# fab-jul/L3C-PyTorch

Measured on AMD Instinct MI355X. Metric: MPix/s encode (net+CDF+AC) on 768x512 RGB, higher is better.
Workload: dtype f32; 1 GPU; L3C 0306_0001 (cr.cf, synthetic seeded checkpoint), batch of 768x512 synthetic RGB per GPU: net forward + fused logistic-mixture CDF head + HIP range coder -> bytes in HBM; checkpoint=calibrated, batch_per_gpu=128, image=768x512, coder_cus=0

## Files before the change

### include/l3c_hip.h

```cpp
#ifndef L3C_HIP_H_
#define L3C_HIP_H_

#include <stdint.h>

#ifdef __cplusplus
extern "C" {
#endif

#define L3C_OK 0
#define L3C_ERR_INVALID_ARG (-1)
#define L3C_ERR_HIP (-2)
#define L3C_ERR_UNSUPPORTED (-3)

#define L3C_ABI_VERSION 4

typedef void *l3c_stream_t;


int l3c_abi_version(void);
#define L3C_BITSTREAM_GENERATION 3
int l3c_bitstream_generation(void);
const char *l3c_last_error(void);
int l3c_device_info(char *name_host, int name_cap, int *num_cu_host, char *arch_host, int arch_cap);

// ... 192 lines not shown
#define L3C_EPI_PIXEL_SHUFFLE 4

typedef struct {
    const float *in;
    int in_cstride, in_coff;
    const float *packed_w;
    const float *bias;
    const float *residual;
    int res_cstride, res_coff;
    float *out;
    int out_cstride, out_coff;
    int B, Hin, Win, Cin, Cout;
    int KS;
    int stride;
    int dilation;
    int epilogue;
} l3c_conv_desc;

int l3c_conv_mfma(const l3c_conv_desc *desc_host, l3c_stream_t stream);
int64_t l3c_conv_wino4_packed_words(int Cout, int Cin);
int l3c_conv_wino4_pack_weights(const float *w_oihw, int Cout, int Cin, float *packed, l3c_stream_t stream);
int l3c_conv_wino4(const l3c_conv_desc *desc_host, l3c_stream_t stream);
int l3c_conv_wino4_phase(const l3c_conv_desc *desc_host, int phase_y, int phase_x, l3c_stream_t stream);
int l3c_conv_wino4_stride2(const l3c_conv_desc *desc_host, l3c_stream_t stream);
int l3c_conv_wino4_set_tiles_per_block(int n);
int64_t l3c_conv_pw_packed_words(int Cout, int Cin);
int l3c_conv_pw_pack_weights(const float *w_oi, int Cout, int Cin, float *packed, l3c_stream_t stream);
int l3c_conv_pw(const l3c_conv_desc *desc_host, l3c_stream_t stream);
int l3c_conv_direct(const l3c_conv_desc *desc_host, l3c_stream_t stream);

int l3c_rgb_head(const float *img, const float *w1, const float *b1, const float *w2, const float *b2,
                 const float *w3, const float *b3, int B, int H, int W, int Cf, float *out, float *shifted_out,
                 l3c_stream_t stream);

int l3c_to_q_quantize(const float *feat, const float *w, const float *b, const float *levels, int64_t B, int64_t HW,
                      int Cf, int C, int L, int16_t *sym, float *bn_q, float *bn, l3c_stream_t stream);

int l3c_dec_head(const float *bn_q, const float *w, const float *b, const float *fuse, int64_t B, int64_t HW, int C,
                 int Cf, float *out, l3c_stream_t stream);

int l3c_meanshift_planar(const float *img, const float *w, const float *b, int64_t B, int64_t HW, float *out,
                         l3c_stream_t stream);
int l3c_rgb_to_u8(const float *x, const float *mean3_host, int64_t B, int64_t HW, uint8_t *out, l3c_stream_t stream);
int l3c_resample_u8(const uint8_t *in, int64_t planes, int H, int W, int axis, int out_size, const int32_t *bounds,
                    const int32_t *kk, int ksize, uint8_t *out, l3c_stream_t stream);
int l3c_u8_to_sym_bn(const uint8_t *in, const float *mean3_host, int64_t B, int64_t HW, int16_t *sym, float *bn,
                     l3c_stream_t stream);

typedef struct {
    const uint8_t *out;
    const uint32_t *nbytes;
    int64_t stride;
    int C, H, W;
} l3c_container_scale;
int l3c_container_write(const l3c_container_scale *scales, int n_scales, int64_t B, const uint16_t *padding,
                        const int64_t *file_offset, uint8_t *dst, l3c_stream_t stream);

int l3c_container_read(const uint8_t *files, const int64_t *src_offset, const int64_t *dst_offset, const uint32_t *nbytes,
                       int64_t n_streams, uint32_t max_nbytes, uint8_t *dst, l3c_stream_t stream);

int l3c_ac_band_intervals(const uint32_t *intervals, int64_t n_streams, int64_t n_sym, int64_t band_len, uint32_t *full_out,
                          uint32_t *last_out, l3c_stream_t stream);

typedef struct {
    const uint8_t *out_full;
    const uint32_t *nbytes_full;
// ... 190 lines not shown
```

### l3c-pytorch_amd/_lib.py

```python
import ctypes
import os

import torch

_HERE = os.path.dirname(os.path.abspath(__file__))
LIB_PATH = os.environ.get('L3C_LIB') or os.path.join(_HERE, 'csrc', 'libl3c_hip.so')

c_i64, c_int, c_vp, c_f32 = ctypes.c_int64, ctypes.c_int, ctypes.c_void_p, ctypes.c_float


class L3CError(RuntimeError):
    pass


class ConvDesc(ctypes.Structure):
    _fields_ = [('inp', c_vp), ('in_cstride', c_int), ('in_coff', c_int),
                ('packed_w', c_vp), ('bias', c_vp),
                ('residual', c_vp), ('res_cstride', c_int), ('res_coff', c_int),
                ('out', c_vp), ('out_cstride', c_int), ('out_coff', c_int),
                ('B', c_int), ('Hin', c_int), ('Win', c_int), ('Cin', c_int), ('Cout', c_int),
                ('KS', c_int), ('stride', c_int), ('dilation', c_int), ('epilogue', c_int)]


class AcGroup(ctypes.Structure):
# ... 141 lines not shown
    'l3c_dmll_cdf_table_parts': (c_int, [c_vp, c_vp, c_vp, c_i64, c_i64, c_int, c_int, c_int, c_int, ctypes.POINTER(TablePart), c_int, c_vp]),
    'l3c_decode_rgb_workspace_bytes': (c_i64, [c_i64, c_i64, c_int, c_int]),
    'l3c_decode_rgb_stats_offset': (c_i64, [c_i64, c_i64, c_int, c_int]),
    'l3c_decode_rgb': (c_int, [ctypes.POINTER(RgbDecodeDesc), c_vp, c_vp]),
    'l3c_decode_rgb_ragged_workspace_bytes': (c_i64, [c_i64, c_i64, c_int, c_int]),
    'l3c_decode_rgb_ragged': (c_int, [ctypes.POINTER(RgbRaggedDesc), c_vp, c_vp]),
    'l3c_dmll_cdf_table_ragged': (c_int, [c_vp, c_vp, c_vp, ctypes.POINTER(RaggedBatch), c_int, c_int, c_int, c_int, ctypes.POINTER(TablePart),
                                          ctypes.POINTER(RaggedPart), c_int, c_vp]),
    'l3c_ac_decode_state_bytes': (c_i64, []),
    'l3c_ac_decode_chunks': (c_int, [ctypes.POINTER(AcDecodePart), c_int, c_vp]),
    'l3c_ac_decode': (c_int, [c_vp, c_i64, c_int, c_vp, c_vp, c_vp, c_i64, c_i64, c_int, c_vp, c_vp]),
    'l3c_cdf_check_monotone': (c_int, [c_vp, c_i64, c_int, c_vp, c_vp]),
    'l3c_dmll_channel_params': (c_int, [c_vp, c_vp, c_i64, c_i64, c_int, c_int, c_int, c_int, c_vp, c_vp, c_vp, c_vp]),
    'l3c_cdf_table_mixture': (c_int, [c_vp, c_vp, c_vp, c_vp, c_i64, c_i64, c_int, c_int, c_vp, c_vp, c_vp]),
    'l3c_dmll_encode_intervals': (c_int, [c_vp, c_vp, c_vp, c_i64, c_i64, c_int, c_int, c_int, c_int, c_vp, c_vp]),
    'l3c_dmll_cdf_table': (c_int, [c_vp, c_vp, c_vp, c_i64, c_i64, c_int, c_int, c_int, c_int, c_i64, c_i64, c_int, c_vp, c_vp, c_vp, c_vp]),
    'l3c_dmll_sample': (c_int, [c_vp, c_vp, c_vp, c_i64, c_i64, c_int, c_int, c_int, c_vp, c_vp]),
    'l3c_dmll_mean': (c_int, [c_vp, c_i64, c_i64, c_int, c_int, c_int, c_f32, c_f32, c_int, c_vp, c_vp]),
    'l3c_dmll_nll': (c_int, [c_vp, c_vp, c_i64, c_i64, c_int, c_int, c_int, c_f32, c_f32, c_int, c_vp, c_vp]),
    'l3c_conv_packed_words': (c_i64, [c_int, c_int, c_int]),
    'l3c_conv_pack_weights': (c_int, [c_vp, c_int, c_int, c_int, c_vp, c_vp]),
    'l3c_conv_mfma': (c_int, [ctypes.POINTER(ConvDesc), c_vp]),
    'l3c_conv_wino4_packed_words': (c_i64, [c_int, c_int]),
    'l3c_conv_wino4_pack_weights': (c_int, [c_vp, c_int, c_int, c_vp, c_vp]),
    'l3c_conv_wino4': (c_int, [ctypes.POINTER(ConvDesc), c_vp]),
    'l3c_conv_wino4_phase': (c_int, [ctypes.POINTER(ConvDesc), c_int, c_int, c_vp]),
    'l3c_conv_wino4_stride2': (c_int, [ctypes.POINTER(ConvDesc), c_vp]),
    'l3c_conv_wino4_set_tiles_per_block': (c_int, [c_int]),
    'l3c_conv_pw_packed_words': (c_i64, [c_int, c_int]),
    'l3c_conv_pw_pack_weights': (c_int, [c_vp, c_int, c_int, c_vp, c_vp]),
    'l3c_conv_pw': (c_int, [ctypes.POINTER(ConvDesc), c_vp]),
    'l3c_conv_direct': (c_int, [ctypes.POINTER(ConvDesc), c_vp]),
    'l3c_rgb_head': (c_int, [c_vp, c_vp, c_vp, c_vp, c_vp, c_vp, c_vp, c_int, c_int, c_int, c_int, c_vp, c_vp, c_vp]),
    'l3c_to_q_quantize': (c_int, [c_vp, c_vp, c_vp, c_vp, c_i64, c_i64, c_int, c_int, c_int, c_vp, c_vp, c_vp, c_vp]),
    'l3c_dec_head': (c_int, [c_vp, c_vp, c_vp, c_vp, c_i64, c_i64, c_int, c_int, c_vp, c_vp]),
    'l3c_meanshift_planar': (c_int, [c_vp, c_vp, c_vp, c_i64, c_i64, c_vp, c_vp]),
    'l3c_rgb_to_u8': (c_int, [c_vp, ctypes.POINTER(c_f32), c_i64, c_i64, c_vp, c_vp]),
    'l3c_resample_u8': (c_int, [c_vp, c_i64, c_int, c_int, c_int, c_int, c_vp, c_vp, c_int, c_vp, c_vp]),
    'l3c_u8_to_sym_bn': (c_int, [c_vp, ctypes.POINTER(c_f32), c_i64, c_i64, c_vp, c_vp, c_vp]),
    'l3c_sym_to_bn': (c_int, [c_vp, c_i64, c_f32, c_f32, c_vp, c_vp]),
    'l3c_net_param_count': (c_int, [ctypes.POINTER(NetConfig)]),
    'l3c_net_param': (c_int, [ctypes.POINTER(NetConfig), c_int, ctypes.c_char_p, c_int, ctypes.POINTER(c_int), ctypes.POINTER(c_i64)]),
    'l3c_net_packed_bytes': (c_i64, [ctypes.POINTER(NetConfig)]),
    'l3c_net_pack_workspace_bytes': (c_i64, [ctypes.POINTER(NetConfig)]),
    'l3c_net_pack': (c_int, [ctypes.POINTER(NetConfig), ctypes.POINTER(c_vp), c_vp, c_i64, c_vp, c_i64, c_vp]),
    'l3c_net_forward_workspace_bytes': (c_i64, [ctypes.POINTER(NetConfig), c_i64, c_int, c_int]),
    'l3c_net_forward': (c_int, [ctypes.POINTER(NetForwardDesc), c_vp]),
    'l3c_net_get_p_workspace_bytes': (c_i64, [ctypes.POINTER(NetConfig), c_i64, c_int, c_int]),
    'l3c_net_get_p': (c_int, [ctypes.POINTER(NetGetPDesc), c_vp]),
    'l3c_container_layout': (c_int, [ctypes.POINTER(ContainerScale), c_int, c_i64, c_i64, c_vp, c_vp, c_vp]),
    'l3c_sym_to_u8': (c_int, [c_vp, c_i64, c_vp, c_vp]),
    'l3c_encode_file_stride': (c_i64, [ctypes.POINTER(NetConfig), c_int, c_int]),
    'l3c_encode_batch_workspace_bytes': (c_i64, [ctypes.POINTER(NetConfig), c_i64, c_int, c_int]),
    'l3c_encode_batch': (c_int, [ctypes.POINTER(EncodeBatchDesc), c_vp]),
    'l3c_decode_plan_bytes': (c_i64, [ctypes.POINTER(NetConfig), c_i64]),
    'l3c_decode_plan': (c_int, [ctypes.POINTER(NetConfig), c_vp, ctypes.POINTER(c_i64), c_i64, c_vp, c_i64, ctypes.POINTER(c_int),
                                ctypes.POINTER(c_int), c_vp]),
    'l3c_decode_batch_workspace_bytes': (c_i64, [ctypes.POINTER(NetConfig), c_vp]),
    'l3c_decode_batch': (c_int, [ctypes.POINTER(DecodeBatchDesc), c_vp, c_vp]),
    'l3c_ac_decode_bands': (c_int, [c_vp, c_int, c_vp, c_vp, c_vp, c_i64, c_i64, c_i64, c_int, c_vp, c_vp]),
    'l3c_container_layout_banded': (c_int, [ctypes.POINTER(BandedScale), c_int, c_i64, c_i64, c_vp, c_vp, c_vp]),
    'l3c_encode_banded_file_stride': (c_i64, [ctypes.POINTER(NetConfig), c_int, c_int, c_int]),
    'l3c_encode_batch_banded_workspace_bytes': (c_i64, [ctypes.POINTER(NetConfig), c_i64, c_int, c_int, c_int]),
    'l3c_encode_batch_banded': (c_int, [ctypes.POINTER(EncodeBatchDesc), c_int, c_vp]),
    'l3c_decode_plan_banded_bytes': (c_i64, [ctypes.POINTER(NetConfig), c_vp, ctypes.POINTER(c_i64), c_i64]),
    'l3c_decode_plan_banded': (c_int, [ctypes.POINTER(NetConfig), c_vp, ctypes.POINTER(c_i64), c_i64, c_vp, c_i64, ctypes.POINTER(c_int),
# ... 135 lines not shown
```

### l3c-pytorch_amd/csrc/conv_small.hip

```cpp
#include "l3c_common.h"

namespace {

typedef float f32x4 __attribute__((ext_vector_type(4)));

constexpr int RH_TH = 8, RH_TW = 32, RH_NT = 4;

__global__ __launch_bounds__(256) void rgb_head_kernel(const float *__restrict__ img, const float *__restrict__ w1,
                                                       const float *__restrict__ b1, const float *__restrict__ w2,
                                                       const float *__restrict__ b2, const float *__restrict__ w3,
                                                       const float *__restrict__ b3, int H, int W, int Cf,
                                                       float *__restrict__ out, float *__restrict__ shifted_out) {
    extern __shared__ __attribute__((aligned(16))) float smem[];
    float *s_w = smem;
    float *s_in = smem + 27 * Cf;
    constexpr int IH = RH_TH + 2, IW = RH_TW + 2;
    const int tid = threadIdx.x;
    const int b = blockIdx.z;
    const int ox0 = blockIdx.x * RH_TW;
    for (int i = tid; i < 27 * Cf; i += 256) {
        const int co = i % Cf, r = i / Cf;
        const int ci = r % 3, tap = r / 3;
        s_w[i] = w3[((size_t)co * 3 + ci) * 9 + tap];
    }
    __syncthreads();
    const int quads = Cf / 4;
    const int q = tid % quads;
    const int pix_per_pass = 256 / quads;
    f32x4 wreg[27];
#pragma unroll
    for (int t = 0; t < 27; ++t) wreg[t] = *reinterpret_cast<const f32x4 *>(&s_w[t * Cf + q * 4]);
    const f32x4 bias = *reinterpret_cast<const f32x4 *>(&b3[q * 4]);
    const size_t plane = (size_t)H * W;
    const float *im = img + (size_t)b * 3 * plane;
    const int Hb = H, Wb = W;
    if (ox0 >= Wb) return;
    for (int nt = 0; nt < RH_NT; ++nt) {
        const int oy0 = (blockIdx.y * RH_NT + nt) * RH_TH;
        if (oy0 >= Hb) break;
        if (nt) __syncthreads();
        for (int i = tid; i < IH * IW; i += 256) {
            const int r = i / IW, c = i % IW;
            const int y = oy0 + r - 1, x = ox0 + c - 1;
            float z[3] = {0.f, 0.f, 0.f};
            if (y >= 0 && y < Hb && x >= 0 && x < Wb) {
                float v[3], u[3];
#pragma unroll
                for (int k = 0; k < 3; ++k) v[k] = im[k * plane + (size_t)y * W + x];
#pragma unroll
                for (int o = 0; o < 3; ++o) u[o] = ((v[0] * w1[o * 3 + 0] + v[1] * w1[o * 3 + 1]) + v[2] * w1[o * 3 + 2]) + b1[o];
#pragma unroll
                for (int o = 0; o < 3; ++o) z[o] = ((u[0] * w2[o * 3 + 0] + u[1] * w2[o * 3 + 1]) + u[2] * w2[o * 3 + 2]) + b2[o];
                if (shifted_out && r >= 1 && r <= RH_TH && c >= 1 && c <= RH_TW) {
#pragma unroll
                    for (int o = 0; o < 3; ++o) shifted_out[((size_t)b * 3 + o) * plane + (size_t)y * W + x] = z[o];
                }
            }
#pragma unroll
            for (int o = 0; o < 3; ++o) s_in[(o * IH + r) * IW + c] = z[o];
        }
        __syncthreads();
        for (int pp = tid / quads; pp < RH_TH * RH_TW; pp += pix_per_pass) {
            const int r = pp / RH_TW, c = pp % RH_TW;
            const int y = oy0 + r, x = ox0 + c;
            if (y >= Hb || x >= Wb) continue;
            f32x4 acc = {0.f, 0.f, 0.f, 0.f};
#pragma unroll
            for (int ky = 0; ky < 3; ++ky)
#pragma unroll
                for (int kx = 0; kx < 3; ++kx)
#pragma unroll
                    for (int ci = 0; ci < 3; ++ci) {
                        const float v = s_in[(ci * IH + r + ky) * IW + c + kx];
                        const f32x4 wq = wreg[(ky * 3 + kx) * 3 + ci];
#pragma unroll
                        for (int e = 0; e < 4; ++e) acc[e] = __builtin_fmaf(v, wq[e], acc[e]);
                    }
            *reinterpret_cast<f32x4 *>(&out[(((size_t)b * H + y) * W + x) * Cf + q * 4]) = acc + bias;
        }
    }
}

__global__ __launch_bounds__(256) void to_q_quantize_kernel(const float *__restrict__ feat, const float *__restrict__ w,
                                                            const float *__restrict__ bias, const float *__restrict__ levels,
                                                            int64_t B, int64_t HW, int Cf, int C, int L,
                                                            int16_t *__restrict__ sym, float *__restrict__ bn_q,
                                                            float *__restrict__ bn) {
    const int64_t total = B * HW;
    for (int64_t i = (int64_t)blockIdx.x * blockDim.x + threadIdx.x; i < total; i += (int64_t)gridDim.x * blockDim.x) {
        const int64_t b = i / HW, n = i % HW;
        const f32x4 *px = reinterpret_cast<const f32x4 *>(feat + i * Cf);
        float acc[8];
#pragma unroll
        for (int c = 0; c < 8; ++c) acc[c] = 0.0f;
        for (int k4 = 0; k4 < Cf / 4; ++k4) {
            const f32x4 v = px[k4];
#pragma unroll
            for (int c = 0; c < 8; ++c)
                if (c < C) {
                    const float *wc = w + c * Cf + k4 * 4;
                    acc[c] = fmaf(v[3], wc[3], fmaf(v[2], wc[2], fmaf(v[1], wc[1], fmaf(v[0], wc[0], acc[c]))));
                }
        }
#pragma unroll
        for (int c = 0; c < 8; ++c)
            if (c < C) {
                const float x = acc[c] + bias[c];
                int best = 0;
                float dbest = (x - levels[0]) * (x - levels[0]);
                for (int l = 1; l < L; ++l) {
                    const float d = (x - levels[l]) * (x - levels[l]);
// ... 201 lines not shown
        const uint8_t *src = in + pl * H * W;
        int acc = 1 << 21;
        if (axis) {
            for (int t = 0; t < count; ++t) acc += (int)src[(int64_t)(first + t) * W + ox] * k[t];
        } else {
            for (int t = 0; t < count; ++t) acc += (int)src[(int64_t)oy * W + first + t] * k[t];
        }
        acc >>= 22;
        out[i] = (uint8_t)(acc < 0 ? 0 : (acc > 255 ? 255 : acc));
    }
}

__global__ __launch_bounds__(256) void u8_to_sym_bn_kernel(const uint8_t *__restrict__ in, float m0, float m1, float m2,
                                                           int64_t B, int64_t HW, int16_t *__restrict__ sym,
                                                           float *__restrict__ bn) {
    const int64_t total = B * 3 * HW;
    for (int64_t i = (int64_t)blockIdx.x * blockDim.x + threadIdx.x; i < total; i += (int64_t)gridDim.x * blockDim.x) {
        const int c = (int)((i / HW) % 3);
        const int v = in[i];
        sym[i] = (int16_t)v;
        bn[i] = (float)v - (c == 0 ? m0 : c == 1 ? m1 : m2);
    }
}

int grid_1d(int64_t total, int block) {
    int64_t g = (total + block - 1) / block;
    return (int)(g < 1 ? 1 : (g > 8192 ? 8192 : g));
}

}

extern "C" {

int l3c_rgb_head(const float *img, const float *w1, const float *b1, const float *w2, const float *b2, const float *w3,
                 const float *b3, int B, int H, int W, int Cf, float *out, float *shifted_out, l3c_stream_t stream) {
    L3C_REQUIRE(img && w1 && b1 && w2 && b2 && w3 && b3 && out, "null pointer");
    L3C_REQUIRE(B > 0 && B < 65536 && H > 0 && W > 0, "bad shape");
    L3C_REQUIRE(Cf % 4 == 0 && Cf >= 4 && Cf <= 256 && 256 % (Cf / 4) == 0, "Cf must be 4 * a divisor of 256");
    const size_t lds = (size_t)(27 * Cf + 3 * (RH_TH + 2) * (RH_TW + 2)) * sizeof(float);
    const dim3 grid((unsigned)((W + RH_TW - 1) / RH_TW), (unsigned)((H + RH_TH * RH_NT - 1) / (RH_TH * RH_NT)), (unsigned)B);
    hipLaunchKernelGGL(rgb_head_kernel, grid, dim3(256), lds, l3c::as_stream(stream), img, w1, b1, w2, b2, w3, b3, H, W,
                       Cf, out, shifted_out);
    return l3c::check_launch("rgb_head_kernel");
}

int l3c_to_q_quantize(const float *feat, const float *w, const float *b, const float *levels, int64_t B, int64_t HW,
                      int Cf, int C, int L, int16_t *sym, float *bn_q, float *bn, l3c_stream_t stream) {
    L3C_REQUIRE(feat && w && b && levels && sym && bn_q, "null pointer");
    L3C_REQUIRE(B > 0 && HW > 0 && Cf % 4 == 0 && C > 0 && C <= 8 && L > 0 && L <= 32767, "bad shape (C <= 8)");
    L3C_REQUIRE((reinterpret_cast<uintptr_t>(feat) & 15) == 0, "feat must be 16-byte aligned (both kernels read it with 16-byte loads)");
#ifndef L3C_TO_Q_DIRECT
    if (Cf <= TQ_MAX_CF) {
        int64_t tiles = (B * HW + TQ_PIX - 1) / TQ_PIX;
        if (tiles > L3C_TQ_GRID) tiles = L3C_TQ_GRID;
        const dim3 grid((unsigned)tiles), block(TQ_PIX);
        switch (C) {
#define L3C_TQ_CASE(c)                                                                                                                \
    case c:                                                                                                                            \
        hipLaunchKernelGGL(to_q_quantize_tile_kernel<c>, grid, block, 0, l3c::as_stream(stream), feat, w, b, levels, B, HW, Cf, L, sym, \
                           bn_q, bn);                                                                                                 \
        break;
            L3C_TQ_CASE(1) L3C_TQ_CASE(2) L3C_TQ_CASE(3) L3C_TQ_CASE(4) L3C_TQ_CASE(5) L3C_TQ_CASE(6) L3C_TQ_CASE(7) L3C_TQ_CASE(8)
#undef L3C_TQ_CASE
        }
        return l3c::check_launch("to_q_quantize_tile_kernel");
    }
#endif
    hipLaunchKernelGGL(to_q_quantize_kernel, dim3(grid_1d(B * HW, 256)), dim3(256), 0, l3c::as_stream(stream), feat, w, b,
                       levels, B, HW, Cf, C, L, sym, bn_q, bn);
    return l3c::check_launch("to_q_quantize_kernel");
}

int l3c_dec_head(const float *bn_q, const float *w, const float *b, const float *fuse, int64_t B, int64_t HW, int C,
                 int Cf, float *out, l3c_stream_t stream) {
    L3C_REQUIRE(bn_q && w && b && out, "null pointer");
    L3C_REQUIRE(B > 0 && B < 65536 && HW > 0 && HW < (1ll << 31) && C > 0 && C <= DH_MAX_C, "bad shape (C <= 8, one image < 2^31 pixels)");
// ... 61 lines not shown
```

### l3c-pytorch_amd/csrc/net.hip

```cpp
#include <string.h>

#include <string>
#include <vector>

#include "l3c_common.h"

#define NET_FAIL(code, ...) (snprintf(l3c::error_buffer(), 512, __VA_ARGS__), (code))

namespace {

constexpr int64_t NET_ALIGN = 256;
constexpr int MAX_BLOCKS = 64;
inline int64_t align_up(int64_t x) { return (x + NET_ALIGN - 1) / NET_ALIGN * NET_ALIGN; }
inline bool aligned16(const void *p) { return (reinterpret_cast<uintptr_t>(p) & 15) == 0; }

int grid_for(int64_t total) {
    const int64_t g = (total + 255) / 256;
    return (int)(g < 1 ? 1 : (g > 4096 ? 4096 : g));
}

__global__ __launch_bounds__(256) void image_symbols_kernel(const float *__restrict__ img, int64_t n, int16_t *__restrict__ sym) {
    for (int64_t i = (int64_t)blockIdx.x * blockDim.x + threadIdx.x; i < n; i += (int64_t)gridDim.x * blockDim.x)
        sym[i] = (int16_t)(long long)rintf(img[i]);
}

__global__ __launch_bounds__(256) void polyphase_concat_kernel(const float *__restrict__ w, int Cout, int Cin, float *__restrict__ w_cat) {
    const int64_t total = (int64_t)Cout * 4 * Cin * 9;
    for (int64_t i = (int64_t)blockIdx.x * blockDim.x + threadIdx.x; i < total; i += (int64_t)gridDim.x * blockDim.x) {
        const int uv = (int)(i % 9);
        const int k = (int)((i / 9) % (4 * Cin));
        const int64_t co = i / (9 * 4 * (int64_t)Cin);
        const int ph = k / Cin, ci = k % Cin;
        const int y = 2 * (uv / 3) + (ph >> 1), x = 2 * (uv % 3) + (ph & 1);
        w_cat[i] = (y <= 4 && x <= 4) ? w[((co * Cin + ci) * 5 + y) * 5 + x] : 0.f;
    }
}

__global__ __launch_bounds__(256) void subpixel_rows_kernel(const float *__restrict__ w, int Cout, int row_len, float *__restrict__ out) {
    const int64_t total = (int64_t)Cout * row_len;
    const int c4 = Cout / 4;
    for (int64_t i = (int64_t)blockIdx.x * blockDim.x + threadIdx.x; i < total; i += (int64_t)gridDim.x * blockDim.x) {
        const int r = (int)(i / row_len);
        const int64_t e = i % row_len;
        out[i] = w[(int64_t)((r % c4) * 4 + r / c4) * row_len + e];
    }
}


struct Param {
    std::string name;
    int ndim;
    int64_t shape[4];
};

int kp_of(const l3c_net_config &c, int s) {
    const int Cp = (c.rgb_baseline || s == 0) ? 3 : c.C;
// ... 349 lines not shown

int l3c_net_forward(const l3c_net_forward_desc *d, l3c_stream_t stream) {
    L3C_REQUIRE(d, "null descriptor");
    NET_TRY(check_config(d->cfg_host, true));
    const l3c_net_config &c = *d->cfg_host;
    if (c.rgb_baseline)
        return NET_FAIL(L3C_ERR_UNSUPPORTED, "l3c_net_forward of an RGB baseline: its bicubic pyramid is driven by host-side resampling "
                        "tables (use l3c_net_get_p for its decoders)");
    const int S = c.num_scales;
    L3C_REQUIRE(d->packed && d->img, "null pointer");
    for (int s = 0; s <= S; ++s) L3C_REQUIRE(d->sym[s] && (s == 0 || d->bn_q[s]) && (s == S || d->P[s]), "null pointer: outputs");
    bool ok = aligned16(d->packed) && aligned16(d->img) && aligned16(d->workspace);
    for (int s = 0; s <= S; ++s) {
        ok = ok && aligned16(d->sym[s]) && aligned16(d->bn_q[s]);
        if (s < S) ok = ok && aligned16(d->P[s]) && aligned16(d->F_enc[s]) && aligned16(d->F_dec[s]);
    }
    L3C_REQUIRE(ok, "every pointer must be 16-byte aligned");
    NET_TRY(check_image(c, d->B, d->H, d->W));
    if (d->H % (1 << S) || d->W % (1 << S))
        return NET_FAIL(L3C_ERR_UNSUPPORTED, "unsupported shape: %d x %d, H and W must be multiples of 2^num_scales = %d", d->H, d->W, 1 << S);
    Layout L;
    build_layout(c, L);
    if (d->packed_bytes != L.bytes)
        return NET_FAIL(L3C_ERR_INVALID_ARG, "packed_bytes %lld != l3c_net_packed_bytes %lld (packed for another config?)",
                        (long long)d->packed_bytes, (long long)L.bytes);
    const FwdPlan p = fwd_plan(c, d->B, d->H, d->W);
    L3C_REQUIRE(d->workspace || p.bytes == 0, "null pointer: workspace");
    if (d->workspace_bytes < p.bytes)
        return NET_FAIL(L3C_ERR_INVALID_ARG, "workspace_bytes too small: %lld < %lld", (long long)d->workspace_bytes, (long long)p.bytes);

    const Run r{static_cast<const char *>(d->packed), &L, (int)d->B, stream};
    const int B = (int)d->B, Cf = c.Cf;
    char *ws = static_cast<char *>(d->workspace);
    const int64_t n_img = (int64_t)B * 3 * d->H * d->W;
    hipLaunchKernelGGL(image_symbols_kernel, dim3(grid_for(n_img)), dim3(256), 0, l3c::as_stream(stream), d->img, n_img, d->sym[0]);
    NET_TRY(l3c::check_launch("image_symbols_kernel"));

    float *A = reinterpret_cast<float *>(ws);
    float *eb[4];
    for (int i = 0; i < 4; ++i) eb[i] = reinterpret_cast<float *>(ws + p.enc_a + i * p.enc_body);
    NET_TRY(l3c_rgb_head(d->img, r.w(L.ms1), r.b(L.ms1), r.w(L.ms2), r.b(L.ms2), r.w(L.head0), r.b(L.head0), B, d->H, d->W, Cf, A,
                         nullptr, stream));
    const float *F_prev = nullptr;
    for (int s = 0; s < S; ++s) {
        const int H = d->H >> s, W = d->W >> s;
        if (s) NET_TRY(conv3(r, L.heads[s], F_prev, Cf, H, W, A, Cf, 0, 1, 0, nullptr, 0));
        l3c_conv_desc dd{};
        dd.in = A;  dd.in_cstride = Cf;  dd.in_coff = 0;
        dd.packed_w = r.w(L.down[s]);  dd.bias = r.b(L.down[s]);
        dd.residual = nullptr;  dd.res_cstride = 0;  dd.res_coff = 0;
        dd.out = eb[0];  dd.out_cstride = Cf;  dd.out_coff = 0;
        dd.B = B;  dd.Hin = H;  dd.Win = W;  dd.Cin = Cf;  dd.Cout = Cf;
        dd.KS = 5;  dd.stride = 2;  dd.dilation = 1;  dd.epilogue = 0;
        NET_TRY(l3c_conv_wino4_stride2(&dd, stream));
        float *F = d->F_enc[s] ? d->F_enc[s] : eb[3];
        NET_TRY(body(r, L.enc_body[s], c.enc_blocks, Cf, H / 2, W / 2, eb[0], eb[1], eb[2], eb[3], F));
        NET_TRY(l3c_to_q_quantize(F, r.w(L.to_q[s]), r.b(L.to_q[s]), r.w(L.levels[s]), B, (int64_t)(H / 2) * (W / 2), Cf, c.C, c.L,
                                  d->sym[s + 1], d->bn_q[s + 1], nullptr, stream));
        F_prev = F;
    }
    float *fd[L3C_NET_MAX_SCALES];
    for (int s = 0; s < S; ++s)
        fd[s] = d->F_dec[s] ? d->F_dec[s] : p.fd_off[s] >= 0 ? reinterpret_cast<float *>(ws + p.fd_off[s]) : d->P[0];
    for (int s = S - 1; s >= 0; --s) {
        const int H = d->H >> (s + 1), W = d->W >> (s + 1);
        NET_TRY(decoder(r, c, s, d->bn_q[s + 1], s == S - 1 ? nullptr : fd[s + 1], H, W, A, (int64_t)B * H * W * Cf, fd[s]));
    }
    for (int s = 0; s < S; ++s) NET_TRY(prob(r, c, s, fd[s], d->H >> s, d->W >> s, A, d->P[s]));
    return L3C_OK;
}

int64_t l3c_net_get_p_workspace_bytes(const l3c_net_config *cfg, int64_t B, int h, int w) {
    NET_TRY(check_config(cfg, true));
    NET_TRY(check_image(*cfg, B, 2ll * h, 2ll * w));
    int64_t m = 0;
// ... 36 lines not shown
```

### l3c-pytorch_amd/modules/multiscale_network.py

```python
import itertools

import numpy as np
import torch
from torch import nn

from .. import ops
from .. import _lib
from ..criterion.logistic_mixture import DiscretizedMixLogisticLoss
from . import schema
from .net import EncOut


class Out(object):

    def __init__(self, targets_style='S', auto_recursive_from=None):
        assert targets_style in ('S', 'bn'), targets_style
        self.S, self.L, self.bn, self.P = [], [], [], []
        self.auto_recursive_from = auto_recursive_from
        self.targets_style = targets_style
        self.raw = _Raw()

    def append(self, enc_out, P, is_training=False):
        self.S.append(enc_out.S)
        self.L.append(enc_out.L)
        self.P.append(P)
        self.bn.append(enc_out.bn if is_training else enc_out.bn_q)
        assert len(self.S) == len(self.L) == len(self.bn) == len(self.P) + 1

    def append_input_image(self, x):
        self.S.append(x.round().long())
        self.L.append(256)
        self.bn.append(None)

    def get_uniform_P(self):
        N, C, H, W = self.S[-1].shape
        return torch.ones(N, self.L[-1], C, H, W, dtype=torch.float32, device=self.S[-1].device)

    def iter_all_scales(self):
        return zip(self.S[1:], self.bn[1:], self.P[1:] + [self.get_uniform_P()], self.L[1:])

    def iter_targets_and_predictions(self, loss_rgb, loss_others):
        yield (loss_rgb, self.S[0].float(), self.P[0])
        other_targets = (S.float() for S in self.S[1:]) if self.targets_style == 'S' else self.bn[1:]
        for t in zip(itertools.repeat(loss_others), other_targets, self.P[1:]):
            yield t

    def get_nat_count(self, i):
        N, C, H, W = self.S[i].shape
        return N * C * H * W * np.log(self.L[i])


class _Raw(object):
    def __init__(self):
        self.sym = []
        self.P = []
        self.bn_q = []
        self.F_enc = []
        self.F_dec = []


class Losses(nn.Module):

    def __init__(self, config_ms):
# ... 113 lines not shown
        return ops.conv(x, tail, residual=skip)

    def _encoder(self, inp, s, pk, want_bn=False):
        e = pk['enc'][s]
        x = ops.conv(inp, e['down'])
        F = self._body(x, e['blocks'], e['tail'])
        q = ops.to_q_quantize(F, e['to_q'][0], e['to_q'][1], e['levels'], want_bn=want_bn)
        return (F,) + tuple(q)

    def _decoder(self, bn_q, fuse, s, pk):
        d = pk['dec'][s]
        x = ops.dec_head(bn_q, d['head'][0], d['head'][1], fuse)
        x = self._body(x, d['blocks'], d['tail'])
        return ops.conv(x, d['up'], pixel_shuffle=True)

    def _prob(self, F, s, pk):
        pr = pk['prob'][s]
        B, H, W, Cf = F.shape
        cat = torch.empty(B, H, W, 3 * Cf, dtype=torch.float32, device=F.device)
        for i, a in enumerate(pr['atrous']):
            ops.conv(F, a, out=cat, out_coff=i * Cf)
        return ops.conv(cat, pr['lin'])


    def forward(self, x, auto_recurse=0):
        _lib.require_gpu()
        x = self._as_device_image(x)
        pk = self._prepare()
        if self._rgb:
            return self._forward_rgb(x, auto_recurse, pk)
        if auto_recurse:
            raise NotImplementedError('auto_recurse is only used by the RGB Shared baseline')
        out = Out(targets_style='bn', auto_recursive_from=None)
        out.append_input_image(x)
        raw = out.raw
        raw.sym.append(out.S[0].to(torch.int16))
        raw.bn_q.append(None)

        inp = ops.rgb_head(x, pk['ms1'][0], pk['ms1'][1], pk['ms2'][0], pk['ms2'][1], pk['head0'][0], pk['head0'][1])
        enc = []
        for s in range(self.scales):
            if s:
                inp = ops.conv(enc[-1][0], pk['heads'][s])
            enc.append(self._encoder(inp, s, pk))
        dec = [None] * self.scales
        for s in reversed(range(self.scales)):
            fuse = None if s == self.scales - 1 else dec[s + 1]
            dec[s] = self._decoder(enc[s][2], fuse, s, pk)
        for s in range(self.scales):
            F, sym, bn_q = enc[s]
            P = self._prob(dec[s], s, pk)
            raw.sym.append(sym)
            raw.bn_q.append(bn_q)
            raw.P.append(P)
            raw.F_enc.append(F)
            raw.F_dec.append(dec[s])
            out.append(EncOut(bn_q, bn_q, sym.long(), self.config_ms.q.L, F.permute(0, 3, 1, 2)), P.permute(0, 3, 1, 2))
        return out

    def _forward_rgb(self, x, auto_recurse, pk):
        forward_scales = list(range(self.scales)) + [-1] * auto_recurse
        out = Out(targets_style='S', auto_recursive_from=self.scales if auto_recurse > 0 else None)
        out.append_input_image(x)
        raw = out.raw
        raw.sym.append(out.S[0].to(torch.int16))
        raw.bn_q.append(None)
        inp = ops.meanshift_planar(x, pk['ms1'][0], pk['ms1'][1])
        encs = []
        for _ in forward_scales:
            bn, sym = ops.bicubic_encoder(inp)
            encs.append((bn, sym))
            inp = bn
# ... 109 lines not shown
```

### l3c-pytorch_amd/ops.py

```python
import ctypes
import os

import numpy as np
import torch

from . import _lib
from ._lib import ConvDesc, call, ptr, stream

PROFILE = None
PROFILE_DETAIL = bool(os.environ.get('L3C_PROFILE_DETAIL'))




class PackedConv(object):

    def __init__(self, weight, bias, stride=1, dilation=1):
        _lib.require_gpu()
        lib = _lib.load()
        self.Cout, self.Cin, self.KS, _ = weight.shape
        self.stride, self.dilation = stride, dilation
        self.weight = weight.detach().to('cuda', torch.float32).contiguous()
        self.bias = bias.detach().to('cuda', torch.float32).contiguous()
        self.packed = None
# ... 127 lines not shown
    call(entry, d, stream())
    e1.record()
    key = ('conv_wino4_kernel' if kernel == 'wino4' else 'conv_lds_kernel<3,{}>'.format(layer.dilation) if layer.KS == 3 else
           'conv k{} s{} (mfma)'.format(layer.KS, layer.stride))
    if PROFILE_DETAIL:
        key += ' {}->{} {}x{}{}{}'.format(layer.Cin, layer.Cout, Ho, Wo, ' +res' if residual is not None else '', ' shuffle' if pixel_shuffle else '')
    nbytes = 4.0 * B * (H * W * layer.Cin + Ho * Wo * layer.Cout * (2 if residual is not None else 1))
    variant = '{},{},{},false'.format(*('true' if f else 'false' for f in (relu, residual is not None, pixel_shuffle))) if kernel == 'wino4' else ''
    PROFILE.append((key, 2.0 * B * Ho * Wo * layer.Cout * layer.Cin * layer.KS * layer.KS, nbytes, e0, e1, variant))
    return out


def _conv_poly5(x, layer, out, in_coff, out_coff, fused=True):
    B, H, W, cstride = x.shape
    e0 = e1 = None
    if PROFILE is not None:
        e0, e1 = torch.cuda.Event(enable_timing=True), torch.cuda.Event(enable_timing=True)
        e0.record()
    if fused:
        d = _conv_desc(x, layer, out, in_coff, out_coff, layer.packed_poly_fused, (5, 2, 1))
        call('l3c_conv_wino4_stride2', d, stream())
    for k, (a, b) in enumerate(() if fused else ((0, 0), (0, 1), (1, 0), (1, 1))):
        packed_w = layer.packed_poly()[k]
        d = _conv_desc(x, layer, out, in_coff, out_coff, packed_w, (3, 2, 1), bias=layer.bias if k == 0 else layer._zero_bias,
                       residual=out if k else None, res_coff=out_coff if k else 0, epilogue=_lib.EPI_RESIDUAL if k else 0)
        call('l3c_conv_wino4_phase', d, a, b, stream())
    if PROFILE is not None:
        e1.record()
        nbytes = 4.0 * B * (H * W * layer.Cin + (H // 2) * (W // 2) * layer.Cout)
        PROFILE.append(('conv k5 s2 (4 F(4x4,3x3) phases)', 2.0 * B * (H // 2) * (W // 2) * layer.Cout * layer.Cin * 25, nbytes, e0, e1))
    return out


def rgb_head(img, ms1_w, ms1_b, ms2_w, ms2_b, conv_w, conv_b, want_shifted=False):
    B, _, H, W = img.shape
    Cf = conv_w.shape[0]
    out = torch.empty(B, H, W, Cf, dtype=torch.float32, device=img.device)
    shifted = torch.empty_like(img) if want_shifted else None
    call('l3c_rgb_head', ptr(img, torch.float32), ptr(ms1_w), ptr(ms1_b), ptr(ms2_w), ptr(ms2_b), ptr(conv_w),
         ptr(conv_b), B, H, W, Cf, ptr(out), ptr(shifted), stream())
    return (out, shifted) if want_shifted else out


def to_q_quantize(feat, w, b, levels, want_bn=False):
    B, H, W, Cf = feat.shape
    C, L = w.shape[0], levels.shape[0]
    sym = torch.empty(B, C, H, W, dtype=torch.int16, device=feat.device)
    bn_q = torch.empty(B, C, H, W, dtype=torch.float32, device=feat.device)
    bn = torch.empty_like(bn_q) if want_bn else None
    call('l3c_to_q_quantize', ptr(feat, torch.float32), ptr(w), ptr(b), ptr(levels), B, H * W, Cf, C, L, ptr(sym),
         ptr(bn_q), ptr(bn), stream())
    return (sym, bn_q, bn) if want_bn else (sym, bn_q)


def dec_head(bn_q, w, b, fuse=None):
    B, C, H, W = bn_q.shape
    Cf = w.shape[0]
    out = torch.empty(B, H, W, Cf, dtype=torch.float32, device=bn_q.device)
    call('l3c_dec_head', ptr(bn_q, torch.float32), ptr(w), ptr(b), ptr(fuse, torch.float32) if fuse is not None else None,
         B, H * W, C, Cf, ptr(out), stream())
    return out


def sym_to_bn(sym, bin_width, x_min):
    bn = torch.empty(sym.shape, dtype=torch.float32, device=sym.device)
    call('l3c_sym_to_bn', ptr(sym, torch.int16), sym.numel(), float(bin_width), float(x_min), ptr(bn), stream())
    return bn



_RGB_MEAN = None
_COEFFS = {}


# ... 445 lines not shown
```

Measured before the change: 186.9 MPix/s.

## Add MFMA RGB head kernel with prefetch and fused image-symbol output

Adds a specialized Cf=64 RGB head kernel that computes the 3x3 conv using 16x16x4 f32 MFMA instructions. It double-buffers the staged tile in LDS and prefetches the next tile's pixels into registers while computing, and stages outputs through LDS so stores are coalesced. It also fuses the image-to-int16 symbol rounding into the head kernel, which removes the separate image_symbols kernel launch and its extra read of the image. In exchange, register pressure goes up and the code becomes more complex. Shapes other than Cf=64 still use the generic kernel.

```diff
diff --git a/include/l3c_hip.h b/include/l3c_hip.h
--- a/include/l3c_hip.h
+++ b/include/l3c_hip.h
@@ -248,6 +248,9 @@
 int l3c_rgb_head(const float *img, const float *w1, const float *b1, const float *w2, const float *b2,
                  const float *w3, const float *b3, int B, int H, int W, int Cf, float *out, float *shifted_out,
                  l3c_stream_t stream);
+int l3c_rgb_head_sym(const float *img, const float *w1, const float *b1, const float *w2, const float *b2,
+                     const float *w3, const float *b3, int B, int H, int W, int Cf, float *out, float *shifted_out,
+                     int16_t *sym_out, l3c_stream_t stream);
 
 int l3c_to_q_quantize(const float *feat, const float *w, const float *b, const float *levels, int64_t B, int64_t HW,
                       int Cf, int C, int L, int16_t *sym, float *bn_q, float *bn, l3c_stream_t stream);
diff --git a/l3c-pytorch_amd/_lib.py b/l3c-pytorch_amd/_lib.py
--- a/l3c-pytorch_amd/_lib.py
+++ b/l3c-pytorch_amd/_lib.py
@@ -197,6 +197,7 @@
     'l3c_conv_pw': (c_int, [ctypes.POINTER(ConvDesc), c_vp]),
     'l3c_conv_direct': (c_int, [ctypes.POINTER(ConvDesc), c_vp]),
     'l3c_rgb_head': (c_int, [c_vp, c_vp, c_vp, c_vp, c_vp, c_vp, c_vp, c_int, c_int, c_int, c_int, c_vp, c_vp, c_vp]),
+    'l3c_rgb_head_sym': (c_int, [c_vp, c_vp, c_vp, c_vp, c_vp, c_vp, c_vp, c_int, c_int, c_int, c_int, c_vp, c_vp, c_vp, c_vp]),
     'l3c_to_q_quantize': (c_int, [c_vp, c_vp, c_vp, c_vp, c_i64, c_i64, c_int, c_int, c_int, c_vp, c_vp, c_vp, c_vp]),
     'l3c_dec_head': (c_int, [c_vp, c_vp, c_vp, c_vp, c_i64, c_i64, c_int, c_int, c_vp, c_vp]),
     'l3c_meanshift_planar': (c_int, [c_vp, c_vp, c_vp, c_i64, c_i64, c_vp, c_vp]),
diff --git a/l3c-pytorch_amd/csrc/conv_small.hip b/l3c-pytorch_amd/csrc/conv_small.hip
--- a/l3c-pytorch_amd/csrc/conv_small.hip
+++ b/l3c-pytorch_amd/csrc/conv_small.hip
@@ -5,16 +5,90 @@
 typedef float f32x4 __attribute__((ext_vector_type(4)));
 
 constexpr int RH_TH = 8, RH_TW = 32, RH_NT = 4;
+
+constexpr int RH_IH = RH_TH + 2, RH_IW = RH_TW + 2;
+
+static_assert(RH_IH * RH_IW <= 512, "two staged positions per thread");
+
+__device__ __forceinline__ void rh_load_pos(const float *__restrict__ im, int Hb, int Wb, size_t plane, int oy0, int ox0, int i,
+                                            float (&v)[3]) {
+    constexpr int IH = RH_IH, IW = RH_IW;
+    const int W = Wb;
+    const int r = i / IW, c = i % IW;
+    const int y = oy0 + r - 1, x = ox0 + c - 1;
+    if (i < IH * IW && y >= 0 && y < Hb && x >= 0 && x < Wb) {
+#pragma unroll
+        for (int k = 0; k < 3; ++k) v[k] = im[k * plane + (size_t)y * W + x];
+    }
+}
+
+__device__ __forceinline__ void rh_finish_pos(const float (&v)[3], const float *__restrict__ w1, const float *__restrict__ b1,
+                                              const float *__restrict__ w2, const float *__restrict__ b2, int Hb, int Wb, size_t plane,
+                                              int oy0, int ox0, int i, float *__restrict__ s_in, float *__restrict__ shifted_b,
+                                              int16_t *__restrict__ sym_b) {
+    constexpr int IH = RH_IH, IW = RH_IW;
+    const int W = Wb;
+    if (i >= IH * IW) return;
+    const int r = i / IW, c = i % IW;
+    const int y = oy0 + r - 1, x = ox0 + c - 1;
+    float z[3] = {0.f, 0.f, 0.f};
+    if (y >= 0 && y < Hb && x >= 0 && x < Wb) {
+        float u[3];
+#pragma unroll
+        for (int o = 0; o < 3; ++o) u[o] = ((v[0] * w1[o * 3 + 0] + v[1] * w1[o * 3 + 1]) + v[2] * w1[o * 3 + 2]) + b1[o];
+#pragma unroll
+        for (int o = 0; o < 3; ++o) z[o] = ((u[0] * w2[o * 3 + 0] + u[1] * w2[o * 3 + 1]) + u[2] * w2[o * 3 + 2]) + b2[o];
+        if (r >= 1 && r <= RH_TH && c >= 1 && c <= RH_TW) {
+            if (shifted_b) {
+#pragma unroll
+                for (int o = 0; o < 3; ++o) shifted_b[o * plane + (size_t)y * W + x] = z[o];
+            }
+            if (sym_b) {
+#pragma unroll
+                for (int k = 0; k < 3; ++k) sym_b[k * plane + (size_t)y * W + x] = (int16_t)(int)rintf(v[k]);
+            }
+        }
+    }
+#pragma unroll
+    for (int o = 0; o < 3; ++o) s_in[(o * IH + r) * IW + c] = z[o];
+}
+
+__device__ __forceinline__ void rh_load_tile(const float *__restrict__ im, int Hb, int Wb, size_t plane, int oy0, int ox0, int tid,
+                                             float (&v)[2][3]) {
+#pragma unroll
+    for (int j = 0; j < 2; ++j) rh_load_pos(im, Hb, Wb, plane, oy0, ox0, tid + j * 256, v[j]);
+}
+
+__device__ __forceinline__ void rh_finish_tile(const float (&v)[2][3], const float *__restrict__ w1, const float *__restrict__ b1,
+                                               const float *__restrict__ w2, const float *__restrict__ b2, int Hb, int Wb, size_t plane,
+                                               int oy0, int ox0, int tid, float *__restrict__ s_in, float *__restrict__ shifted_b,
+                                               int16_t *__restrict__ sym_b) {
+#pragma unroll
+    for (int j = 0; j < 2; ++j) rh_finish_pos(v[j], w1, b1, w2, b2, Hb, Wb, plane, oy0, ox0, tid + j * 256, s_in, shifted_b, sym_b);
+}
+
+__device__ __forceinline__ void rh_stage_tile(const float *__restrict__ im, const float *__restrict__ w1, const float *__restrict__ b1,
+                                              const float *__restrict__ w2, const float *__restrict__ b2, int Hb, int Wb, size_t plane,
+                                              int oy0, int ox0, int tid, float *__restrict__ s_in, float *__restrict__ shifted_b,
+                                              int16_t *__restrict__ sym_b) {
+#pragma unroll 1
+    for (int i = tid; i < RH_IH * RH_IW; i += 256) {
+        float v[3];
+        rh_load_pos(im, Hb, Wb, plane, oy0, ox0, i, v);
+        rh_finish_pos(v, w1, b1, w2, b2, Hb, Wb, plane, oy0, ox0, i, s_in, shifted_b, sym_b);
+    }
+}
 
 __global__ __launch_bounds__(256) void rgb_head_kernel(const float *__restrict__ img, const float *__restrict__ w1,
                                                        const float *__restrict__ b1, const float *__restrict__ w2,
                                                        const float *__restrict__ b2, const float *__restrict__ w3,
                                                        const float *__restrict__ b3, int H, int W, int Cf,
-                                                       float *__restrict__ out, float *__restrict__ shifted_out) {
+                                                       float *__restrict__ out, float *__restrict__ shifted_out,
+                                                       int16_t *__restrict__ sym_out) {
     extern __shared__ __attribute__((aligned(16))) float smem[];
     float *s_w = smem;
     float *s_in = smem + 27 * Cf;
-    constexpr int IH = RH_TH + 2, IW = RH_TW + 2;
+    constexpr int IH = RH_IH, IW = RH_IW;
     const int tid = threadIdx.x;
     const int b = blockIdx.z;
     const int ox0 = blockIdx.x * RH_TW;
@@ -33,32 +107,15 @@
     const f32x4 bias = *reinterpret_cast<const f32x4 *>(&b3[q * 4]);
     const size_t plane = (size_t)H * W;
     const float *im = img + (size_t)b * 3 * plane;
+    float *shifted_b = shifted_out ? shifted_out + (size_t)b * 3 * plane : nullptr;
+    int16_t *sym_b = sym_out ? sym_out + (size_t)b * 3 * plane : nullptr;
     const int Hb = H, Wb = W;
     if (ox0 >= Wb) return;
     for (int nt = 0; nt < RH_NT; ++nt) {
         const int oy0 = (blockIdx.y * RH_NT + nt) * RH_TH;
         if (oy0 >= Hb) break;
         if (nt) __syncthreads();
-        for (int i = tid; i < IH * IW; i += 256) {
-            const int r = i / IW, c = i % IW;
-            const int y = oy0 + r - 1, x = ox0 + c - 1;
-            float z[3] = {0.f, 0.f, 0.f};
-            if (y >= 0 && y < Hb && x >= 0 && x < Wb) {
-                float v[3], u[3];
-#pragma unroll
-                for (int k = 0; k < 3; ++k) v[k] = im[k * plane + (size_t)y * W + x];
-#pragma unroll
-                for (int o = 0; o < 3; ++o) u[o] = ((v[0] * w1[o * 3 + 0] + v[1] * w1[o * 3 + 1]) + v[2] * w1[o * 3 + 2]) + b1[o];
-#pragma unroll
-                for (int o = 0; o < 3; ++o) z[o] = ((u[0] * w2[o * 3 + 0] + u[1] * w2[o * 3 + 1]) + u[2] * w2[o * 3 + 2]) + b2[o];
-                if (shifted_out && r >= 1 && r <= RH_TH && c >= 1 && c <= RH_TW) {
-#pragma unroll
-                    for (int o = 0; o < 3; ++o) shifted_out[((size_t)b * 3 + o) * plane + (size_t)y * W + x] = z[o];
-                }
-            }
-#pragma unroll
-            for (int o = 0; o < 3; ++o) s_in[(o * IH + r) * IW + c] = z[o];
-        }
+        rh_stage_tile(im, w1, b1, w2, b2, Hb, Wb, plane, oy0, ox0, tid, s_in, shifted_b, sym_b);
         __syncthreads();
         for (int pp = tid / quads; pp < RH_TH * RH_TW; pp += pix_per_pass) {
             const int r = pp / RH_TW, c = pp % RH_TW;
@@ -77,6 +134,85 @@
                         for (int e = 0; e < 4; ++e) acc[e] = __builtin_fmaf(v, wq[e], acc[e]);
                     }
             *reinterpret_cast<f32x4 *>(&out[(((size_t)b * H + y) * W + x) * Cf + q * 4]) = acc + bias;
+        }
+    }
+}
+
+constexpr int RH_CF = 64;
+constexpr int RH_OS = RH_CF + 4;
+
+__global__ __launch_bounds__(256) __attribute__((amdgpu_waves_per_eu(5)))
+void rgb_head_kernel_mfma(const float *__restrict__ img, const float *__restrict__ w1, const float *__restrict__ b1,
+                          const float *__restrict__ w2, const float *__restrict__ b2, const float *__restrict__ w3,
+                          const float *__restrict__ b3, int H, int W, float *__restrict__ out, float *__restrict__ shifted_out,
+                          int16_t *__restrict__ sym_out) {
+    constexpr int IH = RH_IH, IW = RH_IW, NCT = RH_CF / 16;
+    __shared__ float s_in2[2][3 * IH * IW];
+    __shared__ __attribute__((aligned(16))) float s_out[4][16 * RH_OS];
+    const int tid = threadIdx.x;
+    const int wave = __builtin_amdgcn_readfirstlane(tid >> 6);
+    const int n = tid & 15, kq = (tid & 63) >> 4;
+    const int b = blockIdx.z;
+    const int ox0 = blockIdx.x * RH_TW;
+    const size_t plane = (size_t)H * W;
+    const float *im = img + (size_t)b * 3 * plane;
+    float *shifted_b = shifted_out ? shifted_out + (size_t)b * 3 * plane : nullptr;
+    int16_t *sym_b = sym_out ? sym_out + (size_t)b * 3 * plane : nullptr;
+    const int Hb = H, Wb = W;
+    const int ty0 = blockIdx.y * RH_NT * RH_TH;
+    if (ox0 >= Wb || ty0 >= Hb) return;
+    float pv[2][3];
+    rh_load_tile(im, Hb, Wb, plane, ty0, ox0, tid, pv);
+    float wa[7][NCT];
+    int toff[7];
+#pragma unroll
+    for (int ks = 0; ks < 7; ++ks) {
+        const int t = ks * 4 + kq;
+        const bool pad = t >= 27;
+        const int tt = pad ? 0 : t;
+        const int ci = tt % 3, tap = tt / 3;
+        toff[ks] = (ci * IH + tap / 3) * IW + tap % 3 + n;
+#pragma unroll
+        for (int ct = 0; ct < NCT; ++ct) wa[ks][ct] = pad ? 0.f : w3[((size_t)(ct * 16 + n) * 3 + ci) * 9 + tap];
+    }
+    const f32x4 bias = *reinterpret_cast<const f32x4 *>(&b3[n * 4]);
+    float *s_o = s_out[wave];
+    for (int nt = 0; nt < RH_NT; ++nt) {
+        const int oy0 = ty0 + nt * RH_TH;
+        if (oy0 >= Hb) break;
+        float *s_in = s_in2[nt & 1];
+        rh_finish_tile(pv, w1, b1, w2, b2, Hb, Wb, plane, oy0, ox0, tid, s_in, shifted_b, sym_b);
+        __syncthreads();
+        if (nt + 1 < RH_NT && oy0 + RH_TH < Hb)
+            rh_load_tile(im, Hb, Wb, plane, oy0 + RH_TH, ox0, tid, pv);
+#pragma unroll
+        for (int i = 0; i < 4; ++i) {
+            const int g = i * 4 + wave;
+            const int r = g >> 1, c0 = (g & 1) * 16;
+            const int y = oy0 + r, x0 = ox0 + c0;
+            if (y >= Hb || x0 >= Wb) continue;
+            const float *s_g = s_in + r * IW + c0;
+            f32x4 acc[NCT];
+#pragma unroll
+            for (int ct = 0; ct < NCT; ++ct) acc[ct] = f32x4{0.f, 0.f, 0.f, 0.f};
+#pragma unroll
+            for (int ks = 0; ks < 7; ++ks) {
+                float v = s_g[toff[ks]];
+                if (ks == 6) v = kq == 3 ? 0.f : v;
+#pragma unroll
+                for (int ct = 0; ct < NCT; ++ct) acc[ct] = __builtin_amdgcn_mfma_f32_16x16x4f32(wa[ks][ct], v, acc[ct], 0, 0, 0);
+            }
+#pragma unroll
+            for (int ct = 0; ct < NCT; ++ct) *reinterpret_cast<f32x4 *>(&s_o[n * RH_OS + ct * 16 + kq * 4]) = acc[ct];
+            __builtin_amdgcn_wave_barrier();
+            float *o = out + (((size_t)b * H + y) * W + x0) * RH_CF + n * 4;
+#pragma unroll
+            for (int j = 0; j < 4; ++j) {
+                const int px = j * 4 + kq;
+                const f32x4 d = *reinterpret_cast<const f32x4 *>(&s_o[px * RH_OS + n * 4]);
+                if (x0 + px < Wb) *reinterpret_cast<f32x4 *>(o + (size_t)px * RH_CF) = d + bias;
+            }
+            __builtin_amdgcn_wave_barrier();
         }
     }
 }
@@ -344,16 +480,28 @@
 
 extern "C" {
 
-int l3c_rgb_head(const float *img, const float *w1, const float *b1, const float *w2, const float *b2, const float *w3,
-                 const float *b3, int B, int H, int W, int Cf, float *out, float *shifted_out, l3c_stream_t stream) {
+int l3c_rgb_head_sym(const float *img, const float *w1, const float *b1, const float *w2, const float *b2, const float *w3,
+                     const float *b3, int B, int H, int W, int Cf, float *out, float *shifted_out, int16_t *sym_out,
+                     l3c_stream_t stream) {
     L3C_REQUIRE(img && w1 && b1 && w2 && b2 && w3 && b3 && out, "null pointer");
     L3C_REQUIRE(B > 0 && B < 65536 && H > 0 && W > 0, "bad shape");
     L3C_REQUIRE(Cf % 4 == 0 && Cf >= 4 && Cf <= 256 && 256 % (Cf / 4) == 0, "Cf must be 4 * a divisor of 256");
-    const size_t lds = (size_t)(27 * Cf + 3 * (RH_TH + 2) * (RH_TW + 2)) * sizeof(float);
+    if (Cf == RH_CF) {
+        const dim3 grid((unsigned)((W + RH_TW - 1) / RH_TW), (unsigned)((H + RH_TH * RH_NT - 1) / (RH_TH * RH_NT)), (unsigned)B);
+        hipLaunchKernelGGL(rgb_head_kernel_mfma, grid, dim3(256), 0, l3c::as_stream(stream), img, w1, b1, w2, b2, w3, b3, H, W,
+                           out, shifted_out, sym_out);
+        return l3c::check_launch("rgb_head_kernel_mfma");
+    }
+    const size_t lds = (size_t)(27 * Cf + 3 * RH_IH * RH_IW) * sizeof(float);
     const dim3 grid((unsigned)((W + RH_TW - 1) / RH_TW), (unsigned)((H + RH_TH * RH_NT - 1) / (RH_TH * RH_NT)), (unsigned)B);
     hipLaunchKernelGGL(rgb_head_kernel, grid, dim3(256), lds, l3c::as_stream(stream), img, w1, b1, w2, b2, w3, b3, H, W,
-                       Cf, out, shifted_out);
+                       Cf, out, shifted_out, sym_out);
     return l3c::check_launch("rgb_head_kernel");
+}
+
+int l3c_rgb_head(const float *img, const float *w1, const float *b1, const float *w2, const float *b2, const float *w3,
+                 const float *b3, int B, int H, int W, int Cf, float *out, float *shifted_out, l3c_stream_t stream) {
+    return l3c_rgb_head_sym(img, w1, b1, w2, b2, w3, b3, B, H, W, Cf, out, shifted_out, nullptr, stream);
 }
 
 int l3c_to_q_quantize(const float *feat, const float *w, const float *b, const float *levels, int64_t B, int64_t HW,
diff --git a/l3c-pytorch_amd/csrc/net.hip b/l3c-pytorch_amd/csrc/net.hip
--- a/l3c-pytorch_amd/csrc/net.hip
+++ b/l3c-pytorch_amd/csrc/net.hip
@@ -17,11 +17,6 @@
 int grid_for(int64_t total) {
     const int64_t g = (total + 255) / 256;
     return (int)(g < 1 ? 1 : (g > 4096 ? 4096 : g));
-}
-
-__global__ __launch_bounds__(256) void image_symbols_kernel(const float *__restrict__ img, int64_t n, int16_t *__restrict__ sym) {
-    for (int64_t i = (int64_t)blockIdx.x * blockDim.x + threadIdx.x; i < n; i += (int64_t)gridDim.x * blockDim.x)
-        sym[i] = (int16_t)(long long)rintf(img[i]);
 }
 
 __global__ __launch_bounds__(256) void polyphase_concat_kernel(const float *__restrict__ w, int Cout, int Cin, float *__restrict__ w_cat) {
@@ -437,15 +432,12 @@
     const Run r{static_cast<const char *>(d->packed), &L, (int)d->B, stream};
     const int B = (int)d->B, Cf = c.Cf;
     char *ws = static_cast<char *>(d->workspace);
-    const int64_t n_img = (int64_t)B * 3 * d->H * d->W;
-    hipLaunchKernelGGL(image_symbols_kernel, dim3(grid_for(n_img)), dim3(256), 0, l3c::as_stream(stream), d->img, n_img, d->sym[0]);
-    NET_TRY(l3c::check_launch("image_symbols_kernel"));
 
     float *A = reinterpret_cast<float *>(ws);
     float *eb[4];
     for (int i = 0; i < 4; ++i) eb[i] = reinterpret_cast<float *>(ws + p.enc_a + i * p.enc_body);
-    NET_TRY(l3c_rgb_head(d->img, r.w(L.ms1), r.b(L.ms1), r.w(L.ms2), r.b(L.ms2), r.w(L.head0), r.b(L.head0), B, d->H, d->W, Cf, A,
-                         nullptr, stream));
+    NET_TRY(l3c_rgb_head_sym(d->img, r.w(L.ms1), r.b(L.ms1), r.w(L.ms2), r.b(L.ms2), r.w(L.head0), r.b(L.head0), B, d->H, d->W, Cf, A,
+                             nullptr, d->sym[0], stream));
     const float *F_prev = nullptr;
     for (int s = 0; s < S; ++s) {
         const int H = d->H >> s, W = d->W >> s;
diff --git a/l3c-pytorch_amd/modules/multiscale_network.py b/l3c-pytorch_amd/modules/multiscale_network.py
--- a/l3c-pytorch_amd/modules/multiscale_network.py
+++ b/l3c-pytorch_amd/modules/multiscale_network.py
@@ -27,8 +27,8 @@
         self.bn.append(enc_out.bn if is_training else enc_out.bn_q)
         assert len(self.S) == len(self.L) == len(self.bn) == len(self.P) + 1
 
-    def append_input_image(self, x):
-        self.S.append(x.round().long())
+    def append_input_image(self, x, sym=None):
+        self.S.append(x.round().long() if sym is None else sym.long())
         self.L.append(256)
         self.bn.append(None)
 
@@ -208,12 +208,12 @@
         if auto_recurse:
             raise NotImplementedError('auto_recurse is only used by the RGB Shared baseline')
         out = Out(targets_style='bn', auto_recursive_from=None)
-        out.append_input_image(x)
+        inp, sym0 = ops.rgb_head(x, pk['ms1'][0], pk['ms1'][1], pk['ms2'][0], pk['ms2'][1], pk['head0'][0], pk['head0'][1], want_sym=True)
+        out.append_input_image(x, sym=sym0)
         raw = out.raw
-        raw.sym.append(out.S[0].to(torch.int16))
+        raw.sym.append(sym0)
         raw.bn_q.append(None)
 
-        inp = ops.rgb_head(x, pk['ms1'][0], pk['ms1'][1], pk['ms2'][0], pk['ms2'][1], pk['head0'][0], pk['head0'][1])
         enc = []
         for s in range(self.scales):
             if s:
diff --git a/l3c-pytorch_amd/ops.py b/l3c-pytorch_amd/ops.py
--- a/l3c-pytorch_amd/ops.py
+++ b/l3c-pytorch_amd/ops.py
@@ -183,14 +183,16 @@
     return out
 
 
-def rgb_head(img, ms1_w, ms1_b, ms2_w, ms2_b, conv_w, conv_b, want_shifted=False):
+def rgb_head(img, ms1_w, ms1_b, ms2_w, ms2_b, conv_w, conv_b, want_shifted=False, want_sym=False):
     B, _, H, W = img.shape
     Cf = conv_w.shape[0]
     out = torch.empty(B, H, W, Cf, dtype=torch.float32, device=img.device)
     shifted = torch.empty_like(img) if want_shifted else None
-    call('l3c_rgb_head', ptr(img, torch.float32), ptr(ms1_w), ptr(ms1_b), ptr(ms2_w), ptr(ms2_b), ptr(conv_w),
-         ptr(conv_b), B, H, W, Cf, ptr(out), ptr(shifted), stream())
-    return (out, shifted) if want_shifted else out
+    sym = torch.empty(B, 3, H, W, dtype=torch.int16, device=img.device) if want_sym else None
+    call('l3c_rgb_head_sym', ptr(img, torch.float32), ptr(ms1_w), ptr(ms1_b), ptr(ms2_w), ptr(ms2_b), ptr(conv_w),
+         ptr(conv_b), B, H, W, Cf, ptr(out), ptr(shifted), ptr(sym), stream())
+    res = (out,) + ((shifted,) if want_shifted else ()) + ((sym,) if want_sym else ())
+    return res if len(res) > 1 else out
 
 
 def to_q_quantize(feat, w, b, levels, want_bn=False):
```

New measurement: 187.3 MPix/s (median of 6 runs). No clear change (+0.2%).
